# chen-bowen/instacart_next_order_recommendation

Hardware: AMD Instinct MI355X
Metric: recommend_qps_top20_49k7_catalog (higher is better)
Workload: dtype f16x3 (f32 operands split into 2 f16 planes, 3 f16 MFMAs per product, f32 accumulate; fp32-level accuracy)

## Files before the change

### instacart_next_order_recommendation_amd/csrc/encoder.hip

```cpp
#include <stdlib.h>

#include <mutex>
#include <type_traits>
#include <vector>

#include "common.h"
#include "wt_gemm.h"
#include "encoder_x3.h"

namespace icrec {

__device__ __forceinline__ int find_seq(const int32_t* __restrict__ cu, int n_seqs, int t) {
    int lo = 0, hi = n_seqs;
    while (hi - lo > 1) {
        int mid = (lo + hi) >> 1;
        if (cu[mid] <= t) lo = mid; else hi = mid;
    }
    return lo;
}

template <int H, bool SPLIT>
__device__ __forceinline__ void ln_row(float (&v)[H / 64], const float* __restrict__ g, const float* __restrict__ b,
                                       float eps, float* __restrict__ out, _Float16* __restrict__ oh,
                                       _Float16* __restrict__ ol, int lane) {
    float s = 0.0f;
#pragma unroll
    for (int j = 0; j < H / 64; ++j) s = s + v[j];
    const float mean = wave_sum_f32(s) / (float)H;
    float q = 0.0f;
#pragma unroll
    for (int j = 0; j < H / 64; ++j) {
        float d = v[j] - mean;
        q = fmaf(d, d, q);
    }
    const float var = wave_sum_f32(q) / (float)H;
    const float rstd = 1.0f / sqrtf(var + eps);
#pragma unroll
    for (int j = 0; j < H / 64; ++j) {
        const int i = lane + 64 * j;
        const float y = fmaf((v[j] - mean) * rstd, g[i], b[i]);
        if (SPLIT) {
            _Float16 hi, lo;
            split_act(y, hi, lo);
            oh[i] = hi;
            ol[i] = lo;
        } else {
            out[i] = y;
        }
    }
}

template <int H, bool SPLIT>
__global__ __launch_bounds__(256) void embed_ln_kernel(const int32_t* __restrict__ ids,
                                                       const int32_t* __restrict__ cu, int n_seqs, int T,
                                                       const float* __restrict__ word, const float* __restrict__ pos,
                                                       const float* __restrict__ type, const float* __restrict__ g,
                                                       const float* __restrict__ b, float eps, int vocab, int max_pos,
                                                       float* __restrict__ x, _Float16* __restrict__ xh,
                                                       _Float16* __restrict__ xl) {
    const int lane = threadIdx.x & 63;
    const int t = blockIdx.x * 4 + (threadIdx.x >> 6);
    if (t >= T) return;
    const int s = find_seq(cu, n_seqs, t);
    int id = ids[t];
    id = id < 0 ? 0 : (id >= vocab ? vocab - 1 : id);
    int p = t - cu[s];
    p = p >= max_pos ? max_pos - 1 : p;
    float v[H / 64];
#pragma unroll
    for (int j = 0; j < H / 64; ++j) {
        const int i = lane + 64 * j;
        v[j] = (word[(size_t)id * H + i] + type[i]) + pos[(size_t)p * H + i];
    }
    ln_row<H, SPLIT>(v, g, b, eps, x + (size_t)t * H, xh + (size_t)t * H, xl + (size_t)t * H, lane);
}

template <int H>
__global__ __launch_bounds__(256) void add_ln_kernel(const float* __restrict__ a, float* __restrict__ x, int T,
                                                     const float* __restrict__ g, const float* __restrict__ b,
                                                     float eps, _Float16* __restrict__ xh,
                                                     _Float16* __restrict__ xl) {
    const int lane = threadIdx.x & 63;
    const int t = blockIdx.x * 4 + (threadIdx.x >> 6);
    if (t >= T) return;
    float v[H / 64];
#pragma unroll
    for (int j = 0; j < H / 64; ++j) {
        const int i = lane + 64 * j;
        v[j] = a[(size_t)t * H + i] + x[(size_t)t * H + i];
    }
    ln_row<H, false>(v, g, b, eps, x + (size_t)t * H, xh + (size_t)t * H, xl + (size_t)t * H, lane);
}

__device__ __forceinline__ float gelu_erf(float x) { return x * 0.5f * (1.0f + erff(x * 0.70710678118654752440f)); }

template <class Cfg, bool GELU>
__global__ __launch_bounds__(Cfg::THREADS, 2) void linear_kernel(const float* __restrict__ A, int M, int K,
                                                                 const float* __restrict__ W, int N,
                                                                 const float* __restrict__ bias,
                                                                 float* __restrict__ out, int n_tiles_n) {
    __shared__ __attribute__((aligned(16))) float smem[Cfg::LDS_FLOATS];
    float* As = smem;
    float* Bs = smem + Cfg::BM * LDK;
    const int lane = threadIdx.x & 63, wave = threadIdx.x >> 6;
    const int wm = wave / Cfg::WAVES_N, wn = wave % Cfg::WAVES_N;
    const int bid = xcd_remap(blockIdx.x, gridDim.x);
    const int mt = bid / n_tiles_n, nt = bid % n_tiles_n;
    const int64_t m0 = (int64_t)mt * Cfg::BM, n0 = (int64_t)nt * Cfg::BN;
    f32x16 acc[Cfg::TM][Cfg::TN];
    tile_gemm<Cfg>(acc, A, m0, M, W, n0, N, K, As, Bs);
#pragma unroll
    for (int j = 0; j < Cfg::TN; ++j) {
        const int64_t col = n0 + (wn * Cfg::TN + j) * 32 + (lane & 31);
        const float bv = col < N ? bias[col] : 0.0f;
#pragma unroll
        for (int i = 0; i < Cfg::TM; ++i)
#pragma unroll
            for (int e = 0; e < 16; ++e) {
                const int64_t row = m0 + (wm * Cfg::TM + i) * 32 + acc_row(e, lane);
                if (row < M && col < N) {
                    float v = acc[i][j][e] + bv;
                    if (GELU) v = gelu_erf(v);
                    out[row * N + col] = v;
                }
            }
    }
}

constexpr int DH = 32;
constexpr int LDQ = 36;

template <int NKT>
__global__ __launch_bounds__(NKT * 64) void attention_kernel(const float* __restrict__ qkv,
                                                             const int32_t* __restrict__ cu, int heads, int H,
                                                             float scale_log2e, float* __restrict__ ctx,
                                                             _Float16* __restrict__ ch, _Float16* __restrict__ cl) {
    __shared__ __attribute__((aligned(16))) float Ks[NKT * 32 * LDQ];
    __shared__ __attribute__((aligned(16))) float Vs[NKT * 32 * DH];
    __shared__ float Ls[NKT * 32];

    const int tid = threadIdx.x, lane = tid & 63, wave = tid >> 6;
    const int s = blockIdx.x / heads, hd = blockIdx.x % heads;
    const int t0 = cu[s], L = cu[s + 1] - t0;
    const int nkt = (L + 31) >> 5;
    if (nkt > NKT || (NKT > 1 && nkt <= NKT / 2)) return;
    const int qb0 = blockIdx.y * NKT;
    if (qb0 >= nkt) return;
    const int ld = 3 * H;

    for (int id = tid; id < nkt * 32 * 8; id += NKT * 64) {
        const int row = id >> 3, c = id & 7;
        const int rr = row < L ? row : L - 1;
        const float* src = qkv + (size_t)(t0 + rr) * ld + hd * DH + c * 4;
        const float4 kv = *reinterpret_cast<const float4*>(src + H);
        const float4 vv = *reinterpret_cast<const float4*>(src + 2 * H);
        float* kp = Ks + row * LDQ + (c >> 1) * 8 + (c & 1) * 2;
        *reinterpret_cast<float2*>(kp) = make_float2(kv.x, kv.z);
        *reinterpret_cast<float2*>(kp + 4) = make_float2(kv.y, kv.w);
        *reinterpret_cast<float4*>(Vs + row * DH + c * 4) = vv;
    }
    const int r = lane & 31, h = lane >> 5;
    const int qb = qb0 + wave;
    float4 qf[4];
    {
        int qr = qb * 32 + r;
        qr = qr < L ? qr : L - 1;
        const float4* qp = reinterpret_cast<const float4*>(qkv + (size_t)(t0 + qr) * ld + hd * DH);
#pragma unroll
        for (int kq = 0; kq < 4; ++kq) {
            const float4 a = qp[2 * kq], b = qp[2 * kq + 1];
            qf[kq] = h == 0 ? make_float4(a.x, a.z, b.x, b.z) : make_float4(a.y, a.w, b.y, b.w);
        }
    }
    __syncthreads();
    if (qb >= nkt) return;

    f32x16 o;
    if constexpr (NKT > 8) {
    auto score_tile = [&](int kt) {
        f32x16 t;
#pragma unroll
        for (int e = 0; e < 16; ++e) t[e] = 0.0f;
#pragma unroll
        for (int kq = 0; kq < 4; ++kq) {
            const float4 kf = *reinterpret_cast<const float4*>(Ks + (kt * 32 + r) * LDQ + kq * 8 + h * 4);
            t = __builtin_amdgcn_mfma_f32_32x32x2f32(kf.x, qf[kq].x, t, 0, 0, 0);
            t = __builtin_amdgcn_mfma_f32_32x32x2f32(kf.y, qf[kq].y, t, 0, 0, 0);
            t = __builtin_amdgcn_mfma_f32_32x32x2f32(kf.z, qf[kq].z, t, 0, 0, 0);
            t = __builtin_amdgcn_mfma_f32_32x32x2f32(kf.w, qf[kq].w, t, 0, 0, 0);
        }
        const bool last = kt == nkt - 1;
#pragma unroll
        for (int e = 0; e < 16; ++e) {
            float v = t[e] * scale_log2e;
            if (last && kt * 32 + acc_row(e, lane) >= L) v = -INFINITY;
            t[e] = v;
        }
        return t;
    };
    float mx = -INFINITY;
    for (int kt = 0; kt < nkt; ++kt) {
        const f32x16 t = score_tile(kt);
#pragma unroll
        for (int e = 0; e < 16; ++e) mx = fmaxf(mx, t[e]);
    }
    mx = fmaxf(mx, __shfl_xor(mx, 32, 64));
    float lsum = 0.0f;
#pragma unroll
    for (int e = 0; e < 16; ++e) o[e] = 0.0f;
    for (int kt = 0; kt < nkt; ++kt) {
        f32x16 t = score_tile(kt);
#pragma unroll
        for (int e = 0; e < 16; ++e) {
            const float p = __builtin_amdgcn_exp2f(t[e] - mx);
            t[e] = p;
            lsum = lsum + p;
        }
#pragma unroll
        for (int e = 0; e < 16; ++e) {
            const int key = kt * 32 + (e & 3) + 8 * (e >> 2) + 4 * h;
            o = __builtin_amdgcn_mfma_f32_32x32x2f32(t[e], Vs[key * DH + r], o, 0, 0, 0);
        }
    }
    {
        const float other = __shfl_xor(lsum, 32, 64);
        lsum = h == 0 ? lsum + other : other + lsum;
    }
    if (h == 0) Ls[wave * 32 + r] = lsum;
    } else {
    f32x16 sc[NKT];
#pragma unroll
    for (int kt = 0; kt < NKT; ++kt) {
#pragma unroll
        for (int e = 0; e < 16; ++e) sc[kt][e] = 0.0f;
        if (kt < nkt) {
#pragma unroll
            for (int kq = 0; kq < 4; ++kq) {
                const float4 kf = *reinterpret_cast<const float4*>(Ks + (kt * 32 + r) * LDQ + kq * 8 + h * 4);
                sc[kt] = __builtin_amdgcn_mfma_f32_32x32x2f32(kf.x, qf[kq].x, sc[kt], 0, 0, 0);
                sc[kt] = __builtin_amdgcn_mfma_f32_32x32x2f32(kf.y, qf[kq].y, sc[kt], 0, 0, 0);
                sc[kt] = __builtin_amdgcn_mfma_f32_32x32x2f32(kf.z, qf[kq].z, sc[kt], 0, 0, 0);
                sc[kt] = __builtin_amdgcn_mfma_f32_32x32x2f32(kf.w, qf[kq].w, sc[kt], 0, 0, 0);
            }
        }
    }
    float mx = -INFINITY;
#pragma unroll
    for (int kt = 0; kt < NKT; ++kt) {
        if (kt < nkt) {
            const bool last = kt == nkt - 1;
#pragma unroll
            for (int e = 0; e < 16; ++e) {
                float v = sc[kt][e] * scale_log2e;
                if (last && kt * 32 + acc_row(e, lane) >= L) v = -INFINITY;
                sc[kt][e] = v;
                mx = fmaxf(mx, v);
            }
        }
    }
    mx = fmaxf(mx, __shfl_xor(mx, 32, 64));
    float lsum = 0.0f;
#pragma unroll
    for (int kt = 0; kt < NKT; ++kt) {
        if (kt < nkt) {
#pragma unroll
            for (int e = 0; e < 16; ++e) {
                const float p = __builtin_amdgcn_exp2f(sc[kt][e] - mx);
                sc[kt][e] = p;
                lsum = lsum + p;
            }
        }
    }
    {
        const float other = __shfl_xor(lsum, 32, 64);
        lsum = h == 0 ? lsum + other : other + lsum;
    }
    if (h == 0) Ls[wave * 32 + r] = lsum;
#pragma unroll
    for (int e = 0; e < 16; ++e) o[e] = 0.0f;
#pragma unroll
    for (int kt = 0; kt < NKT; ++kt) {
        if (kt < nkt) {
#pragma unroll
            for (int e = 0; e < 16; ++e) {
                const int key = kt * 32 + (e & 3) + 8 * (e >> 2) + 4 * h;
                o = __builtin_amdgcn_mfma_f32_32x32x2f32(sc[kt][e], Vs[key * DH + r], o, 0, 0, 0);
            }
        }
    }
    }
#pragma unroll
    for (int e = 0; e < 16; ++e) {
        const int qrow = acc_row(e, lane);
        const int tq = qb * 32 + qrow;
        if (tq < L) {
            const float v = o[e] / Ls[wave * 32 + qrow];
            ctx[(size_t)(t0 + tq) * H + hd * DH + r] = v;
        }
    }
}

__global__ __launch_bounds__(1024) void seq_order_kernel(const int32_t* __restrict__ cu, int n_seqs,
                                                         int32_t* __restrict__ order) {
    constexpr int NB = ICREC_MAX_SEQLEN / 32;
    __shared__ int hist[NB];
    const int tid = threadIdx.x;
    if (tid < NB) hist[tid] = 0;
    __syncthreads();
    auto bin = [&](int s) {
        const int L = cu[s + 1] - cu[s];
        const int nkt = (L + 31) >> 5;
        return NB - (nkt < 1 ? 1 : (nkt > NB ? NB : nkt));
    };
    for (int s0 = tid; s0 < n_seqs; s0 += 1024) atomicAdd(&hist[bin(n_seqs - 1 - s0)], 1);
    __syncthreads();
    if (tid == 0) {
        int run = 0;
        for (int b = 0; b < NB; ++b) { const int c = hist[b]; hist[b] = run; run += c; }
    }
    __syncthreads();
    for (int s0 = tid; s0 < n_seqs; s0 += 1024) {
        const int s = n_seqs - 1 - s0;
        order[atomicAdd(&hist[bin(s)], 1)] = s;
    }
}

typedef _Float16 half2v __attribute__((ext_vector_type(2)));

__device__ __forceinline__ half4 lds_read_tr(const _Float16* p) {
    typedef __fp16 fp16x4 __attribute__((__vector_size__(4 * sizeof(__fp16))));
    return __builtin_bit_cast(half4, __builtin_amdgcn_ds_read_tr16_b64_v4f16(
                                         (__attribute__((address_space(3))) fp16x4*)(reinterpret_cast<uintptr_t>(p))));
}

template <int NKT>
__global__ __launch_bounds__(NKT * 64, (NKT >= 6 ? 4 : NKT == 4 ? 3 : 1)) void attention_x3_kernel(const float* __restrict__ qkv,
                                                                  const int32_t* __restrict__ cu, int heads, int H,
                                                                  float scale_log2e, float* __restrict__ ctx,
                                                                  _Float16* __restrict__ ch, _Float16* __restrict__ cl,
                                                                  const int32_t* __restrict__ order, int nlo) {
    constexpr bool RECOMP = NKT >= 6;
    __shared__ __attribute__((aligned(16))) _Float16 Kbuf[2 * NKT * 32 * 32];
    _Float16* const Kh = Kbuf;
    _Float16* const Kl = Kbuf + NKT * 32 * 32;
    __shared__ __attribute__((aligned(16))) _Float16 Vh[NKT * 32 * 32];
    __shared__ __attribute__((aligned(16))) _Float16 Vl[NKT * 32 * 32];
    __shared__ float Ls[NKT * 32];
    _Float16* const Ob = Kbuf;

    const int tid = threadIdx.x, lane = tid & 63, wave = tid >> 6;
    const int sidx = blockIdx.x / heads, hd = blockIdx.x % heads;
    const int s = order != nullptr ? order[sidx] : sidx;
    const int t0 = cu[s], L = cu[s + 1] - t0;
    const int nkt = (L + 31) >> 5;
    if (nkt > NKT || nkt <= nlo) return;
    const int qb0 = blockIdx.y * NKT;
    if (qb0 >= nkt) return;
    const int ld = 3 * H;

    const int r = lane & 31, h = lane >> 5;
    const int qb = qb0 + wave;
    half8 qh[2], ql[2];
    {
        int qr = qb * 32 + r;
        qr = qr < L ? qr : L - 1;
        const float* qp = qkv + (size_t)(t0 + qr) * ld + hd * DH;
#pragma unroll
        for (int ks = 0; ks < 2; ++ks) {
            const f32x4 a = *reinterpret_cast<const f32x4*>(qp + 16 * ks + 8 * h);
            const f32x4 b = *reinterpret_cast<const f32x4*>(qp + 16 * ks + 8 * h + 4);
            half4 ah, al, bh, bl;
            split_act4(a, ah, al);
            split_act4(b, bh, bl);
            qh[ks] = half8{ah[0], ah[1], ah[2], ah[3], bh[0], bh[1], bh[2], bh[3]};
            ql[ks] = half8{al[0], al[1], al[2], al[3], bl[0], bl[1], bl[2], bl[3]};
        }
    }
    constexpr int STG = NKT * 32 * 8 / (NKT * 64);
    static_assert(NKT * 32 * 8 % (NKT * 64) == 0, "staging: whole rounds");
    f32x4 kreg[STG], vreg[STG];
#pragma unroll
    for (int it = 0; it < STG; ++it) {
        const int id = tid + it * NKT * 64;
        const int key = id >> 3, c = id & 7;
        const int rr = key < L ? key : L - 1;
        const float* src = qkv + (size_t)(t0 + rr) * ld + hd * DH + c * 4;
        kreg[it] = *reinterpret_cast<const f32x4*>(src + H);
        vreg[it] = *reinterpret_cast<const f32x4*>(src + 2 * H);
    }
#pragma unroll
    for (int it = 0; it < STG; ++it) {
        const int id = tid + it * NKT * 64;
        if (id < nkt * 32 * 8) {
            const int key = id >> 3, c = id & 7;
            half4 khi, klo, vhi, vlo;
            split_act4(kreg[it], khi, klo);
            split_act4(vreg[it], vhi, vlo);
            *reinterpret_cast<half4*>(Vh + key * 32 + c * 4) = vhi;
            *reinterpret_cast<half4*>(Vl + key * 32 + c * 4) = vlo;
            const int off = key * 32 + ((((c >> 1) ^ ((key >> 2) & 3)) << 3) | ((c & 1) << 2));
            *reinterpret_cast<half4*>(Kh + off) = khi;
            *reinterpret_cast<half4*>(Kl + off) = klo;
        }
    }
    __syncthreads();
    const bool active = qb < nkt;

    auto score_tile = [&](int kt, bool hi_only = false) {
        f32x16 t;
#pragma unroll
        for (int e = 0; e < 16; ++e) t[e] = 0.0f;
        const int key = kt * 32 + r;
#pragma unroll
        for (int ks = 0; ks < 2; ++ks) {
            const int off = key * 32 + (((2 * ks + h) ^ ((key >> 2) & 3)) << 3);
            const half8 kh = *reinterpret_cast<const half8*>(Kh + off);
            const half8 kl = *reinterpret_cast<const half8*>(Kl + off);
            t = __builtin_amdgcn_mfma_f32_32x32x16_f16(kh, qh[ks], t, 0, 0, 0);
            if (hi_only) continue;
            t = __builtin_amdgcn_mfma_f32_32x32x16_f16(kh, ql[ks], t, 0, 0, 0);
            t = __builtin_amdgcn_mfma_f32_32x32x16_f16(kl, qh[ks], t, 0, 0, 0);
        }
        if (kt == nkt - 1 && kt * 32 + 32 > L) {
#pragma unroll
            for (int e = 0; e < 16; ++e)
                if (kt * 32 + acc_row(e, lane) >= L) t[e] = -INFINITY;
        }
        return t;
    };
    auto pv_tile = [&](int kt, const f32x16& pt, f32x16& o) {
#pragma unroll
        for (int ks = 0; ks < 2; ++ks) {
            half8 ph, pl;
#pragma unroll
            for (int j = 0; j < 8; j += 2) {
                half2w a, b;
                split_pair_prescaled(pt[8 * ks + j], pt[8 * ks + j + 1], a, b);
                ph[j] = a[0]; ph[j + 1] = a[1];
                pl[j] = b[0]; pl[j + 1] = b[1];
            }
            const int base = kt * 32 + 4 * h + 16 * ks;
            const int tr_at = (base + ((lane & 15) >> 2)) * 32 + 16 * ((lane >> 4) & 1) + 4 * (lane & 3);
            const half4 v0h = lds_read_tr(Vh + tr_at);
            const half4 v1h = lds_read_tr(Vh + tr_at + 8 * 32);
            const half4 v0l = lds_read_tr(Vl + tr_at);
            const half4 v1l = lds_read_tr(Vl + tr_at + 8 * 32);
            const half8 vh = {v0h[0], v0h[1], v0h[2], v0h[3], v1h[0], v1h[1], v1h[2], v1h[3]};
            const half8 vl = {v0l[0], v0l[1], v0l[2], v0l[3], v1l[0], v1l[1], v1l[2], v1l[3]};
            o = __builtin_amdgcn_mfma_f32_32x32x16_f16(ph, vh, o, 0, 0, 0);
            o = __builtin_amdgcn_mfma_f32_32x32x16_f16(ph, vl, o, 0, 0, 0);
            o = __builtin_amdgcn_mfma_f32_32x32x16_f16(pl, vh, o, 0, 0, 0);
        }
    };
    typedef float float2w __attribute__((ext_vector_type(2)));
    const float cs = scale_log2e * (1.0f / 256.0f);
    f32x16 o;
#pragma unroll
    for (int e = 0; e < 16; ++e) o[e] = 0.0f;
    if (RECOMP) {
        if (active) {
            float mx = -INFINITY;
#pragma unroll
            for (int kt = 0; kt < NKT; ++kt) {
                if (kt < nkt) {
                    const f32x16 t = score_tile(kt, true);
#pragma unroll
                    for (int e = 0; e < 16; ++e) mx = fmaxf(mx, t[e]);
                }
            }
            mx = fmaxf(mx, __shfl_xor(mx, 32, 64));
            const float shift = fmaf(-mx, cs, 10.0f);
            float2w ls2 = float2w{0.0f, 0.0f};
#pragma unroll
            for (int kt = 0; kt < NKT; ++kt) {
                if (kt < nkt) {
                    f32x16 t = score_tile(kt);
#pragma unroll
                    for (int e = 0; e < 16; ++e) t[e] = __builtin_amdgcn_exp2f(fminf(fmaf(t[e], cs, shift), 15.9f));
#pragma unroll
                    for (int e = 0; e < 16; e += 2) ls2 = ls2 + float2w{t[e], t[e + 1]};
                    pv_tile(kt, t, o);
                }
            }
            float lrow = ls2[0] + ls2[1];
            const float other = __shfl_xor(lrow, 32, 64);
            lrow = h == 0 ? lrow + other : other + lrow;
            if (h == 0) Ls[wave * 32 + r] = lrow;
        }
    } else {
    if (active) {
    f32x16 sc[NKT];
#pragma unroll
    for (int kt = 0; kt < NKT; ++kt)
        if (kt < nkt) sc[kt] = score_tile(kt);
    float mx = -INFINITY;
#pragma unroll
    for (int kt = 0; kt < NKT; ++kt) {
        if (kt < nkt) {
#pragma unroll
            for (int e = 0; e < 16; ++e) mx = fmaxf(mx, sc[kt][e]);
        }
    }
    mx = fmaxf(mx, __shfl_xor(mx, 32, 64));
    const float shift = fmaf(-mx, cs, 10.0f);
#pragma unroll
    for (int kt = 0; kt < NKT; ++kt) {
        if (kt < nkt) {
#pragma unroll
            for (int e = 0; e < 16; ++e) sc[kt][e] = __builtin_amdgcn_exp2f(fmaf(sc[kt][e], cs, shift));
        }
    }
    float2w ls2 = float2w{0.0f, 0.0f};
#pragma unroll
    for (int kt = 0; kt < NKT; ++kt) {
        if (kt < nkt) {
#pragma unroll
            for (int e = 0; e < 16; e += 2) ls2 = ls2 + float2w{sc[kt][e], sc[kt][e + 1]};
        }
    }
    float lrow = ls2[0] + ls2[1];
    {
        const float other = __shfl_xor(lrow, 32, 64);
        lrow = h == 0 ? lrow + other : other + lrow;
    }
    if (h == 0) Ls[wave * 32 + r] = lrow;

#pragma unroll
    for (int kt = 0; kt < NKT; ++kt)
        if (kt < nkt) pv_tile(kt, sc[kt], o);
    }
    }
    __syncthreads();
    if (!active) return;
    _Float16* ob = Ob + wave * (2 * 32 * 32);
#pragma unroll
    for (int e = 0; e < 16; e += 2) {
        const int q0 = acc_row(e, lane), q1 = acc_row(e + 1, lane);
        const float v0 = o[e] * (0.0625f * __builtin_amdgcn_rcpf(Ls[wave * 32 + q0]));
        const float v1 = o[e + 1] * (0.0625f * __builtin_amdgcn_rcpf(Ls[wave * 32 + q1]));
        half2w hi, lo;
        split_pair_prescaled(v0 * WT_SA, v1 * WT_SA, hi, lo);
        ob[q0 * 32 + r] = hi[0];
        ob[q1 * 32 + r] = hi[1];
        ob[32 * 32 + q0 * 32 + r] = lo[0];
        ob[32 * 32 + q1 * 32 + r] = lo[1];
    }
#pragma unroll
    for (int t = 0; t < 2; ++t) {
        const int id = lane + 64 * t, qrow = id >> 2, c8 = (id & 3) * 8;
        const int tq = qb * 32 + qrow;
        if (tq < L) {
            const size_t at = (size_t)(t0 + tq) * H + hd * DH + c8;
            *reinterpret_cast<u32x4*>(ch + at) = *reinterpret_cast<const u32x4*>(ob + qrow * 32 + c8);
            *reinterpret_cast<u32x4*>(cl + at) = *reinterpret_cast<const u32x4*>(ob + 32 * 32 + qrow * 32 + c8);
        }
    }
}

template <int H, bool PLANES>
__global__ __launch_bounds__(H) void pool_norm_kernel(const float* __restrict__ x, const _Float16* __restrict__ xh,
                                                      const _Float16* __restrict__ xl, const int32_t* __restrict__ cu,
                                                      int n_norm, float* __restrict__ out) {
    auto at = [&](size_t idx) { return PLANES ? ((float)xh[idx] + (float)xl[idx]) * (1.0f / WT_SA) : x[idx]; };
    __shared__ float v[H];
    __shared__ float den_s;
    const int s = blockIdx.x, i = threadIdx.x;
    const int t0 = cu[s], t1 = cu[s + 1];
    float acc = 0.0f;
    int t = t0;
    for (; t + 8 <= t1; t += 8) {
        float v[8];
#pragma unroll
        for (int u = 0; u < 8; ++u) v[u] = at((size_t)(t + u) * H + i);
#pragma unroll
        for (int u = 0; u < 8; ++u) acc = acc + v[u];
    }
    for (; t < t1; ++t) acc = acc + at((size_t)t * H + i);
    float cnt = (float)(t1 - t0);
    cnt = cnt < 1e-9f ? 1e-9f : cnt;
    float val = acc / cnt;
    for (int rep = 0; rep < n_norm; ++rep) {
        v[i] = val;
        __syncthreads();
        if (i < 64) {
            float a = 0.0f;
#pragma unroll
            for (int j = 0; j < H / 64; ++j) a = fmaf(v[i + 64 * j], v[i + 64 * j], a);
            const float nrm = sqrtf(wave_sum_f32(a));
            if (i == 0) den_s = nrm > 1e-12f ? nrm : 1e-12f;
        }
        __syncthreads();
        val = val / den_s;
        __syncthreads();
    }
    out[(size_t)s * H + i] = val;
}

constexpr int HID = 384;

struct LayerW {
    float *Wqkv, *bqkv, *Wo, *bo, *g1, *b1n, *W1, *b1, *W2, *b2, *g2, *b2n;
    _Float16 *Wqkv_p, *Wo_p, *W1_p, *W2_p;
};
struct Encoder {
    icrec_bert_cfg cfg;
    int device = 0;
    int n_cu = 256;
    int max_seqlen = 256;
    float* blob = nullptr;
    float* extra = nullptr;
    _Float16* planes = nullptr;
    float *word, *pos, *type, *eg, *eb;
    LayerW layers[64];
    bool fuse = true, side_stream = true;
    int small_m = 3584;
    int tail_m = 2560;
    struct Side {
        hipStream_t caller = nullptr, side = nullptr;
        hipEvent_t ev = nullptr;
    };
    std::mutex side_mu;
    std::vector<Side*> sides;
};

static int side_for(Encoder* e, hipStream_t caller, Encoder::Side** out) {
    std::lock_guard<std::mutex> lock(e->side_mu);
    *out = nullptr;
    for (Encoder::Side* sd : e->sides)
        if (sd->caller == caller) { *out = sd; return ICREC_OK; }
    hipStreamCaptureStatus cap = hipStreamCaptureStatusNone;
    if (caller && hipStreamIsCapturing(caller, &cap) == hipSuccess && cap != hipStreamCaptureStatusNone)
        return ICREC_OK;
    Encoder::Side* sd = new Encoder::Side();
    sd->caller = caller;
    ICREC_HIP(hipStreamCreateWithFlags(&sd->side, hipStreamNonBlocking));
    ICREC_HIP(hipEventCreateWithFlags(&sd->ev, hipEventDisableTiming));
    e->sides.push_back(sd);
    *out = sd;
    return ICREC_OK;
}

static size_t weight_count(const icrec_bert_cfg* c) {
    const size_t H = c->hidden, I = c->intermediate;
    const size_t emb = (size_t)c->vocab_size * H + (size_t)c->max_position * H + (size_t)c->type_vocab * H + 2 * H;
    const size_t per = 4 * (H * H + H) + 2 * H + (I * H + I) + (H * I + H) + 2 * H;
    return emb + per * c->layers;
}

struct EncWs {
    size_t x, xs, qkv, ctx, t1, h, total;
};
static EncWs enc_ws(const icrec_bert_cfg& c, int64_t T) {
    auto al = [](size_t b) { return (b + 255) & ~(size_t)255; };
    EncWs w;
    size_t o = 0;
    w.x = o;   o += al((size_t)T * c.hidden * 4);
    w.xs = o;  o += al((size_t)T * c.hidden * 4);
    w.qkv = o; o += al((size_t)T * 3 * c.hidden * 4);
    w.ctx = o; o += al((size_t)T * c.hidden * 4);
    w.t1 = o;  o += al((size_t)T * c.hidden * 4);
    w.h = o;   o += al((size_t)T * c.intermediate * 4);
    w.total = o;
    return w;
}

struct EncBufs {
    float *x, *qkv, *ctx, *t1, *h;
    _Float16 *xh, *xl, *ch, *cl, *hh, *hl;
};

typedef TileCfg<2, 2, 2, 2> GemmBig;
constexpr long long SMALL_M_MAX = 1 << 20;

static int env_knob(const char* name, int fallback, long long hi) {
    const char* s = getenv(name);
    if (!s) return fallback;
    char* end = nullptr;
    const long long v = strtoll(s, &end, 10);
    if (end == s) return fallback;
    return (int)(v < 0 ? 0 : v > hi ? hi : v);
}

template <bool GELU>
static void launch_linear(const float* A, int M, int K, const float* W, int N, const float* bias, float* out,
                          hipStream_t st) {
    const int mt = (M + GemmBig::BM - 1) / GemmBig::BM, nt = (N + GemmBig::BN - 1) / GemmBig::BN;
    hipLaunchKernelGGL((linear_kernel<GemmBig, GELU>), dim3(mt * nt), dim3(GemmBig::THREADS), 0, st, A, M, K, W, N,
                       bias, out, nt);
}

template <int EPI>
static void launch_wt_linear(const _Float16* Xh, const _Float16* Xl, int T, int K, const _Float16* Wp, int N,
                             const float* bias, float* out, _Float16* oh, _Float16* ol, hipStream_t st, bool small) {
    if (small) {
        if constexpr (EPI == 0 || EPI == 2) {
            const int nbn = N / 64;
            auto kern = K % 256 == 0 && K >= 1024 ? wt_linear_half_kernel<EPI, 8> : wt_linear_half_kernel<EPI, 6>;
            hipLaunchKernelGGL(kern, dim3(((T + 31) / 32) * nbn), dim3(256), 0, st, Xh, Xl, T, K, Wp, N, bias, out,
                               (const _Float16*)oh, (const _Float16*)ol, nbn);
        } else {
            const int nbn = N / 128;
            hipLaunchKernelGGL((wt_linear_kernel<1, 1, 4, EPI>), dim3(((T + 31) / 32) * nbn), dim3(256), 0, st, Xh, Xl, T, K,
                               Wp, N, bias, out, oh, ol, nbn);
        }
    } else {
        const int nbn = N / 384;
        hipLaunchKernelGGL((wt_linear_kernel<3, 2, 1, EPI>), dim3(((T + 63) / 64) * nbn), dim3(256), 0, st, Xh, Xl, T, K,
                           Wp, N, bias, out, oh, ol, nbn);
    }
}

enum AttBucket { ATT_9_16, ATT_1, ATT_2, ATT_3_4, ATT_5_6, ATT_7_8, ATT_5_8, ATT_N };
constexpr int ATT_LO[ATT_N] = {9, 1, 2, 3, 5, 7, 5}, ATT_HI[ATT_N] = {16, 1, 2, 4, 6, 8, 8};

template <bool X3>
static void launch_attention(unsigned mask, const icrec_bert_cfg& c, const EncBufs& b, const int32_t* cu, int n_seqs,
                             int max_seqlen, const int32_t* order, hipStream_t st) {
    const int nkt_max = (max_seqlen + 31) / 32;
    const bool single = n_seqs == 1, split_5_8 = X3 && !single;
    const float sl2e = (1.0f / sqrtf((float)DH)) * 1.44269504088896340736f;
    for (int k = 0; k < ATT_N; ++k) {
        if (!(mask >> k & 1) || (split_5_8 ? k == ATT_5_8 : k == ATT_5_6 || k == ATT_7_8) || nkt_max < ATT_LO[k] ||
            (single && nkt_max > ATT_HI[k]))
            continue;
        const dim3 grid(n_seqs * c.heads, 1), block(ATT_HI[k] * 64);
        if constexpr (X3) {
            static const decltype(&attention_x3_kernel<1>) kern[ATT_N] = {
                attention_x3_kernel<16>, attention_x3_kernel<1>, attention_x3_kernel<2>, attention_x3_kernel<4>,
                attention_x3_kernel<6>, attention_x3_kernel<8>, attention_x3_kernel<8>};
            hipLaunchKernelGGL(kern[k], grid, block, 0, st, b.qkv, cu, c.heads, c.hidden, sl2e, b.ctx, b.ch, b.cl, order,
                               ATT_LO[k] - 1);
        } else {
            static const decltype(&attention_kernel<1>) kern[ATT_N] = {
                attention_kernel<16>, attention_kernel<1>, attention_kernel<2>, attention_kernel<4>, nullptr, nullptr,
                attention_kernel<8>};
            hipLaunchKernelGGL(kern[k], grid, block, 0, st, b.qkv, cu, c.heads, c.hidden, sl2e, b.ctx, b.ch, b.cl);
        }
    }
}

}

using namespace icrec;

extern "C" {

size_t icrec_encoder_weight_count(const icrec_bert_cfg* cfg) { return cfg ? weight_count(cfg) : 0; }

int icrec_encoder_create(const float* weights_host, size_t n_floats, const icrec_bert_cfg* cfg, int device,
                         icrec_encoder** out) {
    ICREC_REQUIRE(weights_host && cfg && out, "icrec_encoder_create: NULL argument");
    ICREC_REQUIRE(cfg->hidden == HID, "icrec_encoder_create: this build supports hidden=384 only (got %d)", cfg->hidden);
    ICREC_REQUIRE(cfg->heads * DH == cfg->hidden, "icrec_encoder_create: head_dim must be 32 (heads=%d)", cfg->heads);
    ICREC_REQUIRE(cfg->intermediate >= 384 && cfg->intermediate % 384 == 0, "icrec_encoder_create: intermediate size must be a multiple of 384 (got %d)", cfg->intermediate);
    ICREC_REQUIRE(cfg->layers >= 1 && cfg->layers <= 64, "icrec_encoder_create: layers must be in [1,64]");
    ICREC_REQUIRE(cfg->vocab_size >= 1 && cfg->max_position >= 1 && cfg->type_vocab >= 1, "icrec_encoder_create: bad vocab/position sizes");
    ICREC_REQUIRE(cfg->n_normalize >= 0 && cfg->n_normalize <= 4, "icrec_encoder_create: n_normalize must be in [0,4]");
    ICREC_REQUIRE(cfg->gemm_mode == ICREC_GEMM_F32 || cfg->gemm_mode == ICREC_GEMM_F16X3, "icrec_encoder_create: unknown gemm_mode %d", cfg->gemm_mode);
    ICREC_REQUIRE(n_floats == weight_count(cfg), "icrec_encoder_create: weight blob has %zu floats, expected %zu", n_floats, weight_count(cfg));
    ICREC_HIP(hipSetDevice(device));
    hipDeviceProp_t prop;
    ICREC_HIP(hipGetDeviceProperties(&prop, device));
    if (strncmp(prop.gcnArchName, "gfx950", 6) != 0) {
        set_error("icrec_encoder_create: device %d is %s, this library is built for gfx950 only", device, prop.gcnArchName);
        return ICREC_ENODEV;
    }
    Encoder* e = new Encoder();
    e->cfg = *cfg;
    e->device = device;
    e->n_cu = prop.multiProcessorCount > 0 ? prop.multiProcessorCount : 256;
    e->max_seqlen = cfg->max_position < 256 ? cfg->max_position : 256;
    {
        const char* fuse_env = getenv("ICREC_FUSE");
        const char* side_env = getenv("ICREC_SIDE_STREAM");
        e->fuse = !(fuse_env && fuse_env[0] == '0');
        e->small_m = env_knob("ICREC_SMALL_M", e->small_m, SMALL_M_MAX);
        e->tail_m = env_knob("ICREC_TAIL_M", e->tail_m, 64LL * e->n_cu - 1);
        e->side_stream = !(side_env && side_env[0] == '0');
    }
    const size_t H = cfg->hidden, I = cfg->intermediate;
    const size_t mat_per_layer = 3 * H * H + H * H + I * H + H * I;
    const bool x3 = cfg->gemm_mode == ICREC_GEMM_F16X3;
    if (hipMalloc(&e->blob, n_floats * 4) != hipSuccess ||
        hipMalloc(&e->extra, (size_t)cfg->layers * (3 * H * H + 3 * H) * 4) != hipSuccess ||
        (x3 && hipMalloc(&e->planes, (size_t)cfg->layers * mat_per_layer * 2 * sizeof(_Float16)) != hipSuccess)) {
        set_error("icrec_encoder_create: hipMalloc failed");
        if (e->blob) (void)hipFree(e->blob);
        if (e->extra) (void)hipFree(e->extra);
        delete e;
        return ICREC_ENOMEM;
    }
    ICREC_HIP(hipMemcpy(e->blob, weights_host, n_floats * 4, hipMemcpyHostToDevice));
    float* p = e->blob;
    e->word = p; p += (size_t)cfg->vocab_size * H;
    e->pos = p;  p += (size_t)cfg->max_position * H;
    e->type = p; p += (size_t)cfg->type_vocab * H;
    e->eg = p;   p += H;
    e->eb = p;   p += H;
    float* x = e->extra;
    _Float16* pl = e->planes;
    auto pack = [&](const float* w, int N, int K, _Float16*& out) {
        out = pl;
        pl += (size_t)2 * N * K;
        hipLaunchKernelGGL(pack_weights_kernel, dim3(1024), dim3(256), 0, 0, w, N, K, out);
    };
    for (int l = 0; l < cfg->layers; ++l) {
        LayerW& L = e->layers[l];
        L.Wqkv = x; x += 3 * H * H;
        L.bqkv = x; x += 3 * H;
        for (int part = 0; part < 3; ++part) {
            ICREC_HIP(hipMemcpy(L.Wqkv + part * H * H, p, H * H * 4, hipMemcpyDeviceToDevice)); p += H * H;
            ICREC_HIP(hipMemcpy(L.bqkv + part * H, p, H * 4, hipMemcpyDeviceToDevice)); p += H;
        }
        L.Wo = p; p += H * H; L.bo = p; p += H;
        L.g1 = p; p += H; L.b1n = p; p += H;
        L.W1 = p; p += I * H; L.b1 = p; p += I;
        L.W2 = p; p += H * I; L.b2 = p; p += H;
        L.g2 = p; p += H; L.b2n = p; p += H;
        if (x3) {
            pack(L.Wqkv, (int)(3 * H), (int)H, L.Wqkv_p);
            pack(L.Wo, (int)H, (int)H, L.Wo_p);
            pack(L.W1, (int)I, (int)H, L.W1_p);
            pack(L.W2, (int)H, (int)I, L.W2_p);
        }
    }
    ICREC_HIP(hipGetLastError());
    ICREC_HIP(hipDeviceSynchronize());
    *out = reinterpret_cast<icrec_encoder*>(e);
    return ICREC_OK;
}

int icrec_encoder_destroy(icrec_encoder* h) {
    Encoder* e = reinterpret_cast<Encoder*>(h);
    if (!e) return ICREC_OK;
    (void)hipSetDevice(e->device);
    (void)hipFree(e->blob);
    (void)hipFree(e->extra);
    if (e->planes) (void)hipFree(e->planes);
    for (Encoder::Side* sd : e->sides) {
        (void)hipStreamSynchronize(sd->side);
        (void)hipStreamDestroy(sd->side);
        (void)hipEventDestroy(sd->ev);
        delete sd;
    }
    delete e;
    return ICREC_OK;
}

int icrec_encoder_set_max_seqlen(icrec_encoder* h, int32_t max_seqlen) {
    Encoder* e = reinterpret_cast<Encoder*>(h);
    ICREC_REQUIRE(e, "icrec_encoder_set_max_seqlen: NULL encoder");
    const int hi = e->cfg.max_position < ICREC_MAX_SEQLEN ? e->cfg.max_position : ICREC_MAX_SEQLEN;
    ICREC_REQUIRE(max_seqlen >= 1 && max_seqlen <= hi, "icrec_encoder_set_max_seqlen: max_seqlen must be in [1, %d] (got %d)", hi, max_seqlen);
    e->max_seqlen = max_seqlen;
    return ICREC_OK;
}

size_t icrec_encode_workspace_bytes(const icrec_encoder* h, int64_t total_tokens, int32_t n_seqs) {
    const Encoder* e = reinterpret_cast<const Encoder*>(h);
    if (!e || total_tokens < 1 || n_seqs < 1) return 0;
    return enc_ws(e->cfg, total_tokens).total;
}

static int batch_tail(const Encoder* e, int T) {
    const int round_tokens = 64 * e->n_cu;
    return T > round_tokens && T % round_tokens <= e->tail_m ? T % round_tokens : 0;
}

int icrec_encode_batch_split(const icrec_encoder* h, int64_t total_tokens, int64_t* main_tokens, int64_t* tail_tokens) {
    const Encoder* e = reinterpret_cast<const Encoder*>(h);
    ICREC_REQUIRE(e && main_tokens && tail_tokens && total_tokens >= 1 && total_tokens < (1ll << 31), "icrec_encode_batch_split: bad argument");
    *tail_tokens = batch_tail(e, (int)total_tokens);
    *main_tokens = total_tokens - *tail_tokens;
    return ICREC_OK;
}

static const int32_t* embed(const Encoder* e, const EncBufs& b, const int32_t* ids_dev, const int32_t* cu_dev,
                            int n_seqs, int T, hipStream_t st) {
    const icrec_bert_cfg& c = e->cfg;
    const bool x3 = c.gemm_mode == ICREC_GEMM_F16X3;
    int32_t* order = nullptr;
    if (x3 && n_seqs >= 64 && e->fuse) {
        order = reinterpret_cast<int32_t*>(b.x);
        hipLaunchKernelGGL(seq_order_kernel, dim3(1), dim3(1024), 0, st, cu_dev, n_seqs, order);
    }
    hipLaunchKernelGGL((x3 ? embed_ln_kernel<HID, true> : embed_ln_kernel<HID, false>), dim3((T + 3) / 4), dim3(256), 0,
                       st, ids_dev, cu_dev, n_seqs, T, e->word, e->pos, e->type, e->eg, e->eb, c.ln_eps, c.vocab_size,
                       c.max_position, b.x, b.xh, b.xl);
    return order;
}

static hipError_t link(const Encoder::Side* sd, hipStream_t from, hipStream_t to) {
    const hipError_t err = hipEventRecord(sd->ev, from);
    return err != hipSuccess ? err : hipStreamWaitEvent(to, sd->ev, 0);
}

struct Range {
    int r0, n;
    hipStream_t st;
    bool small;
    bool layer;
    bool fold;
    Range(const Encoder* e, int r0, int n, hipStream_t st)
        : r0(r0), n(n), st(st), small(n <= e->small_m), layer(e->fuse && !small), fold(e->fuse && small) {}
    bool launches_qkv(int l) const { return l == 0 || !layer; }
    bool ffn_ln_to_next(int l, int layers) const { return fold && l + 1 < layers; }
};

static int encode_x3(Encoder* e, const EncBufs& b, const int32_t* cu_dev, int n_seqs, int T, int max_seqlen,
                     const int32_t* order, hipStream_t st) {
    const icrec_bert_cfg& c = e->cfg;
    const int H = c.hidden, I = c.intermediate;
    const bool split_att = e->side_stream && n_seqs >= 64 && max_seqlen > 128;
    const int T_tail = batch_tail(e, T), T_main = T - T_tail;
    Encoder::Side* sd = nullptr;
    if (e->side_stream && (T_tail || split_att))
        if (int rc_ = side_for(e, st, &sd)) return rc_;
    const Range main(e, 0, T_main, st), tail(e, T_main, T_tail, sd ? sd->side : st);
    const bool tail_on_side = T_tail && sd;
    if (main.layer || tail.layer) {
        if (int rc_ = ensure_dynamic_lds(reinterpret_cast<const void*>(qkv_resident_kernel), QKVR_LDS)) return rc_;
        if (int rc_ = ensure_dynamic_lds(reinterpret_cast<const void*>(ffn_fused2_kernel), FFN2_LDS)) return rc_;
    }

    auto qkv_stage = [&](const Range& r, int l) {
        const LayerW& L = e->layers[l];
        _Float16 *const xhr = b.xh + (size_t)r.r0 * H, *const xlr = b.xl + (size_t)r.r0 * H;
        float* const qkvr = b.qkv + (size_t)r.r0 * 3 * H;
        if (r.layer) {
            hipLaunchKernelGGL(qkv_resident_kernel, dim3((r.n + 63) / 64), dim3(512), QKVR_LDS, r.st, xhr, xlr, r.n,
                               L.Wqkv_p, L.bqkv, qkvr, 3 * H);
        } else if (l > 0 && r.ffn_ln_to_next(l - 1, c.layers)) {
            const LayerW& Lp = e->layers[l - 1];
            const int nbn = 3 * H / 64;
            hipLaunchKernelGGL((wt_linear_lnin_kernel<0>), dim3(((r.n + 31) / 32) * nbn), dim3(256), 0, r.st,
                               (const float*)(b.t1 + (size_t)r.r0 * H), r.n, Lp.g2, Lp.b2n, c.ln_eps, xhr, xlr, L.Wqkv_p,
                               3 * H, L.bqkv, qkvr, (_Float16*)nullptr, (_Float16*)nullptr, nbn);
        } else {
            launch_wt_linear<0>(xhr, xlr, r.n, H, L.Wqkv_p, 3 * H, L.bqkv, qkvr, nullptr, nullptr, r.st, r.small);
        }
    };
    auto post_stage = [&](const Range& r, int l) {
        const LayerW& L = e->layers[l];
        float* const t1r = b.t1 + (size_t)r.r0 * H;
        _Float16 *const xhr = b.xh + (size_t)r.r0 * H, *const xlr = b.xl + (size_t)r.r0 * H;
        const _Float16 *const chr = b.ch + (size_t)r.r0 * H, *const clr = b.cl + (size_t)r.r0 * H;
        if (r.layer) {
            ScopedTimer tm(T_FFN_UP, r.st);
            const bool next_qkv = l + 1 < c.layers;
            const LayerW& Ln = e->layers[next_qkv ? l + 1 : l];
            hipLaunchKernelGGL(ffn_fused2_kernel, dim3((r.n + 63) / 64), dim3(512), FFN2_LDS, r.st, xhr, xlr, r.n, I,
                               L.W1_p, L.b1, L.W2_p, L.b2, L.g2, L.b2n, c.ln_eps, chr, clr, L.Wo_p, L.bo, L.g1, L.b1n,
                               next_qkv ? (const _Float16*)Ln.Wqkv_p : (const _Float16*)nullptr, (const float*)Ln.bqkv,
                               b.qkv + (size_t)r.r0 * 3 * H, 3 * H);
            return;
        }
        _Float16 *const hhr = b.hh + (size_t)r.r0 * I, *const hlr = b.hl + (size_t)r.r0 * I;
        launch_wt_linear<2>(chr, clr, r.n, H, L.Wo_p, H, L.bo, t1r, xhr, xlr, r.st, r.small);
        if (r.fold) {
            const int nbn = I / 64;
            hipLaunchKernelGGL((wt_linear_lnin_kernel<1>), dim3(((r.n + 31) / 32) * nbn), dim3(256), 0, r.st,
                               (const float*)t1r, r.n, L.g1, L.b1n, c.ln_eps, xhr, xlr, L.W1_p, I, L.b1, (float*)nullptr,
                               hhr, hlr, nbn);
        } else {
            hipLaunchKernelGGL(ln_wt_kernel, dim3((r.n + 15) / 16), dim3(256), 0, r.st, t1r, r.n, L.g1, L.b1n, c.ln_eps,
                               xhr, xlr);
            ScopedTimer tm(r.small ? T_NSLOTS - 1 : T_FFN_UP, r.st);
            launch_wt_linear<1>(xhr, xlr, r.n, H, L.W1_p, I, L.b1, nullptr, hhr, hlr, r.st, r.small);
        }
        launch_wt_linear<2>(hhr, hlr, r.n, I, L.W2_p, H, L.b2, t1r, xhr, xlr, r.st, r.small);
        if (!r.ffn_ln_to_next(l, c.layers))
            hipLaunchKernelGGL(ln_wt_kernel, dim3((r.n + 15) / 16), dim3(256), 0, r.st, t1r, r.n, L.g2, L.b2n, c.ln_eps,
                               xhr, xlr);
    };

    if (tail_on_side) ICREC_HIP(link(sd, st, sd->side));
    for (int l = 0; l < c.layers; ++l) {
        if (T_tail && tail.launches_qkv(l)) qkv_stage(tail, l);
        if (main.launches_qkv(l)) qkv_stage(main, l);
        if (tail_on_side) ICREC_HIP(link(sd, sd->side, st));
        if (split_att && sd) {
            ICREC_HIP(link(sd, st, sd->side));
            const unsigned side_buckets = 1u << ATT_1 | 1u << ATT_2 | 1u << ATT_3_4 | 1u << ATT_7_8;
            launch_attention<true>(1u << ATT_9_16, c, b, cu_dev, n_seqs, max_seqlen, order, st);
            launch_attention<true>(side_buckets, c, b, cu_dev, n_seqs, max_seqlen, order, sd->side);
            launch_attention<true>(1u << ATT_5_6, c, b, cu_dev, n_seqs, max_seqlen, order, st);
            ICREC_HIP(link(sd, sd->side, st));
        } else {
            launch_attention<true>(~0u, c, b, cu_dev, n_seqs, max_seqlen, order, st);
        }
        if (tail_on_side) ICREC_HIP(link(sd, st, sd->side));
        if (T_tail) post_stage(tail, l);
        post_stage(main, l);
    }
    if (tail_on_side) ICREC_HIP(link(sd, sd->side, st));
    return ICREC_OK;
}

static int encode_f32(const Encoder* e, const EncBufs& b, const int32_t* cu_dev, int n_seqs, int T, int max_seqlen,
                      hipStream_t st) {
    const icrec_bert_cfg& c = e->cfg;
    const int H = c.hidden, I = c.intermediate, rows_grid = (T + 3) / 4;
    for (int l = 0; l < c.layers; ++l) {
        const LayerW& L = e->layers[l];
        launch_linear<false>(b.x, T, H, L.Wqkv, 3 * H, L.bqkv, b.qkv, st);
        launch_attention<false>(~0u, c, b, cu_dev, n_seqs, max_seqlen, nullptr, st);
        launch_linear<false>(b.ctx, T, H, L.Wo, H, L.bo, b.t1, st);
        hipLaunchKernelGGL(add_ln_kernel<HID>, dim3(rows_grid), dim3(256), 0, st, b.t1, b.x, T, L.g1, L.b1n,
                           c.ln_eps, b.xh, b.xl);
        {
            ScopedTimer tm(T_FFN_UP, st);
            launch_linear<true>(b.x, T, H, L.W1, I, L.b1, b.h, st);
        }
        launch_linear<false>(b.h, T, I, L.W2, H, L.b2, b.t1, st);
        hipLaunchKernelGGL(add_ln_kernel<HID>, dim3(rows_grid), dim3(256), 0, st, b.t1, b.x, T, L.g2, L.b2n,
                           c.ln_eps, b.xh, b.xl);
    }
    return ICREC_OK;
}

int icrec_encode(icrec_encoder* h, const int32_t* ids_dev, const int32_t* cu_dev, int32_t n_seqs, int64_t T64,
                 int32_t max_seqlen, float* out_dev, void* ws, size_t ws_bytes, void* stream) {
    Encoder* e = reinterpret_cast<Encoder*>(h);
    ICREC_REQUIRE(e && ids_dev && cu_dev && out_dev, "icrec_encode: NULL argument");
    ICREC_REQUIRE(n_seqs >= 1 && T64 >= n_seqs && T64 < (1ll << 31), "icrec_encode: bad n_seqs/total_tokens (%d, %lld)", n_seqs, (long long)T64);
    ICREC_REQUIRE(max_seqlen >= 1 && max_seqlen <= e->max_seqlen, "icrec_encode: max_seqlen must be in [1, %d] (got %d)", e->max_seqlen, max_seqlen);
    const int T = (int)T64;
    const EncWs w = enc_ws(e->cfg, T);
    if (!ws || ws_bytes < w.total) {
        set_error("icrec_encode: workspace too small (%zu < %zu)", ws_bytes, w.total);
        return ICREC_ENOMEM;
    }
    ICREC_HIP(hipSetDevice(e->device));
    hipStream_t st = (hipStream_t)stream;
    ScopedTimer whole(T_ENCODE, st);
    char* base = reinterpret_cast<char*>(ws);
    const icrec_bert_cfg& c = e->cfg;
    const int H = c.hidden, I = c.intermediate;
    const bool x3 = c.gemm_mode == ICREC_GEMM_F16X3;
    EncBufs b;
    b.x = reinterpret_cast<float*>(base + w.x);
    b.qkv = reinterpret_cast<float*>(base + w.qkv);
    b.ctx = reinterpret_cast<float*>(base + w.ctx);
    b.t1 = reinterpret_cast<float*>(base + w.t1);
    b.h = reinterpret_cast<float*>(base + w.h);
    b.xh = reinterpret_cast<_Float16*>(base + w.xs);
    b.xl = b.xh + (size_t)T * H;
    b.ch = reinterpret_cast<_Float16*>(b.ctx);
    b.cl = b.ch + (size_t)T * H;
    b.hh = reinterpret_cast<_Float16*>(b.h);
    b.hl = b.hh + (size_t)T * I;
    const int32_t* order = embed(e, b, ids_dev, cu_dev, n_seqs, T, st);
    if (int rc_ = x3 ? encode_x3(e, b, cu_dev, n_seqs, T, max_seqlen, order, st)
                     : encode_f32(e, b, cu_dev, n_seqs, T, max_seqlen, st))
        return rc_;
    hipLaunchKernelGGL((x3 ? pool_norm_kernel<HID, true> : pool_norm_kernel<HID, false>), dim3(n_seqs), dim3(HID), 0, st,
                       b.x, b.xh, b.xl, cu_dev, c.n_normalize, out_dev);
    ICREC_HIP(hipGetLastError());
    return ICREC_OK;
}

}
```

Measured before the change: 109,200.

## Fuse embedding+LayerNorm into first-layer QKV kernel and overlap seq ordering on side stream

Result: no change. 109,600, median of 6 (+0.4%).

```diff
diff --git a/instacart_next_order_recommendation_amd/csrc/encoder.hip b/instacart_next_order_recommendation_amd/csrc/encoder.hip
--- a/instacart_next_order_recommendation_amd/csrc/encoder.hip
+++ b/instacart_next_order_recommendation_amd/csrc/encoder.hip
@@ -57,9 +57,9 @@
                                                        const float* __restrict__ type, const float* __restrict__ g,
                                                        const float* __restrict__ b, float eps, int vocab, int max_pos,
                                                        float* __restrict__ x, _Float16* __restrict__ xh,
-                                                       _Float16* __restrict__ xl) {
+                                                       _Float16* __restrict__ xl, int t0 = 0) {
     const int lane = threadIdx.x & 63;
-    const int t = blockIdx.x * 4 + (threadIdx.x >> 6);
+    const int t = t0 + blockIdx.x * 4 + (threadIdx.x >> 6);
     if (t >= T) return;
     const int s = find_seq(cu, n_seqs, t);
     int id = ids[t];
@@ -73,6 +73,67 @@
         v[j] = (word[(size_t)id * H + i] + type[i]) + pos[(size_t)p * H + i];
     }
     ln_row<H, SPLIT>(v, g, b, eps, x + (size_t)t * H, xh + (size_t)t * H, xl + (size_t)t * H, lane);
+}
+
+__global__ __launch_bounds__(512, 2) void embed_qkv_kernel(const int32_t* __restrict__ ids,
+                                                           const int32_t* __restrict__ cu, int n_seqs, int T,
+                                                           const float* __restrict__ word, const float* __restrict__ pos,
+                                                           const float* __restrict__ type, const float* __restrict__ eg,
+                                                           const float* __restrict__ eb, float eps, int vocab,
+                                                           int max_pos, _Float16* __restrict__ xh,
+                                                           _Float16* __restrict__ xl, const _Float16* __restrict__ Wp,
+                                                           const float* __restrict__ bias, float* __restrict__ out,
+                                                           int N) {
+    constexpr int H = 384, NTOK = 64 / 8;
+    extern __shared__ __attribute__((aligned(16))) char smem2[];
+    char* const Xs = smem2;
+    const int tid = threadIdx.x, lane = tid & 63, wave = wave_uniform(tid >> 6), c = lane & 15, g = lane >> 4;
+    float* const stg = reinterpret_cast<float*>(smem2 + FFN2_X_BYTES + wave * QKVR_STG_BYTES);
+    const int64_t m0 = (int64_t)blockIdx.x * 64;
+    const int tw = (int)m0 + wave * NTOK;
+    float* const par = reinterpret_cast<float*>(smem2 + FFN2_X_BYTES);
+    if (tid < 192) *reinterpret_cast<f32x4*>(par + 4 * tid) = wt_ln_par_load(eg, eb, tid);
+    int id = 0, p = 0;
+    if (lane < NTOK) {
+        const int t = tw + lane < T ? tw + lane : T - 1;
+        id = ids[t];
+        id = id < 0 ? 0 : (id >= vocab ? vocab - 1 : id);
+        p = t - cu[find_seq(cu, n_seqs, t)];
+        p = p >= max_pos ? max_pos - 1 : p;
+    }
+    float v[NTOK][H / 64];
+#pragma unroll
+    for (int k = 0; k < NTOK; ++k) {
+        const int ik = __builtin_amdgcn_readlane(id, k), pk = __builtin_amdgcn_readlane(p, k);
+#pragma unroll
+        for (int j = 0; j < H / 64; ++j) {
+            const int i = lane + 64 * j;
+            v[k][j] = (word[(size_t)ik * H + i] + type[i]) + pos[(size_t)pk * H + i];
+        }
+    }
+    bar_lds();
+#pragma unroll
+    for (int k = 0; k < NTOK; ++k) {
+        _Float16* const row = reinterpret_cast<_Float16*>(Xs + (wave * NTOK + k) * 768);
+        ln_row<H, true>(v[k], par, par + H, eps, nullptr, row, row + FFN2_XPLANE / 2, lane);
+    }
+    lds_order();
+    constexpr int NR = 2 * NTOK * 48 / 64;
+    u32x4 o[NR];
+#pragma unroll
+    for (int r = 0; r < NR; ++r) {
+        const int idx = lane + 64 * r, pl = idx / (NTOK * 48), k = idx / 48 % NTOK, ch = idx % 48;
+        o[r] = *reinterpret_cast<const u32x4*>(Xs + pl * FFN2_XPLANE + (wave * NTOK + k) * 768 + ch * 16);
+    }
+    lds_order();
+#pragma unroll
+    for (int r = 0; r < NR; ++r) {
+        const int idx = lane + 64 * r, pl = idx / (NTOK * 48), k = idx / 48 % NTOK, ch = idx % 48;
+        *reinterpret_cast<u32x4*>(Xs + pl * FFN2_XPLANE + ffn_x_pos(wave * NTOK + k, ch)) = o[r];
+        if (tw + k < T) *reinterpret_cast<u32x4*>((pl ? xl : xh) + (int64_t)(tw + k) * H + ch * 8) = o[r];
+    }
+    __syncthreads();
+    qkv_block_walk(Xs, stg, Wp, bias, out, N, m0, T, wave, lane, c, g, lane * 8);
 }
 
 template <int H>
@@ -875,19 +936,13 @@
     return ICREC_OK;
 }
 
-static const int32_t* embed(const Encoder* e, const EncBufs& b, const int32_t* ids_dev, const int32_t* cu_dev,
-                            int n_seqs, int T, hipStream_t st) {
+static void embed(const Encoder* e, const EncBufs& b, const int32_t* ids_dev, const int32_t* cu_dev, int n_seqs, int t0,
+                  int T, hipStream_t st) {
     const icrec_bert_cfg& c = e->cfg;
     const bool x3 = c.gemm_mode == ICREC_GEMM_F16X3;
-    int32_t* order = nullptr;
-    if (x3 && n_seqs >= 64 && e->fuse) {
-        order = reinterpret_cast<int32_t*>(b.x);
-        hipLaunchKernelGGL(seq_order_kernel, dim3(1), dim3(1024), 0, st, cu_dev, n_seqs, order);
-    }
-    hipLaunchKernelGGL((x3 ? embed_ln_kernel<HID, true> : embed_ln_kernel<HID, false>), dim3((T + 3) / 4), dim3(256), 0,
-                       st, ids_dev, cu_dev, n_seqs, T, e->word, e->pos, e->type, e->eg, e->eb, c.ln_eps, c.vocab_size,
-                       c.max_position, b.x, b.xh, b.xl);
-    return order;
+    hipLaunchKernelGGL((x3 ? embed_ln_kernel<HID, true> : embed_ln_kernel<HID, false>), dim3((T - t0 + 3) / 4),
+                       dim3(256), 0, st, ids_dev, cu_dev, n_seqs, T, e->word, e->pos, e->type, e->eg, e->eb, c.ln_eps,
+                       c.vocab_size, c.max_position, b.x, b.xh, b.xl, t0);
 }
 
 static hipError_t link(const Encoder::Side* sd, hipStream_t from, hipStream_t to) {
@@ -907,19 +962,23 @@
     bool ffn_ln_to_next(int l, int layers) const { return fold && l + 1 < layers; }
 };
 
-static int encode_x3(Encoder* e, const EncBufs& b, const int32_t* cu_dev, int n_seqs, int T, int max_seqlen,
-                     const int32_t* order, hipStream_t st) {
+static int encode_x3(Encoder* e, const EncBufs& b, const int32_t* ids_dev, const int32_t* cu_dev, int n_seqs, int T,
+                     int max_seqlen, hipStream_t st) {
     const icrec_bert_cfg& c = e->cfg;
     const int H = c.hidden, I = c.intermediate;
     const bool split_att = e->side_stream && n_seqs >= 64 && max_seqlen > 128;
     const int T_tail = batch_tail(e, T), T_main = T - T_tail;
+    const Range main(e, 0, T_main, st);
+    int32_t* const order = e->fuse && n_seqs >= 64 ? reinterpret_cast<int32_t*>(b.x) : nullptr;
     Encoder::Side* sd = nullptr;
-    if (e->side_stream && (T_tail || split_att))
+    if (e->side_stream && (T_tail || split_att || (main.layer && order)))
         if (int rc_ = side_for(e, st, &sd)) return rc_;
-    const Range main(e, 0, T_main, st), tail(e, T_main, T_tail, sd ? sd->side : st);
+    const Range tail(e, T_main, T_tail, sd ? sd->side : st);
     const bool tail_on_side = T_tail && sd;
+    const bool pre_on_side = main.layer && sd;
     if (main.layer || tail.layer) {
         if (int rc_ = ensure_dynamic_lds(reinterpret_cast<const void*>(qkv_resident_kernel), QKVR_LDS)) return rc_;
+        if (int rc_ = ensure_dynamic_lds(reinterpret_cast<const void*>(embed_qkv_kernel), QKVR_LDS)) return rc_;
         if (int rc_ = ensure_dynamic_lds(reinterpret_cast<const void*>(ffn_fused2_kernel), FFN2_LDS)) return rc_;
     }
 
@@ -927,7 +986,11 @@
         const LayerW& L = e->layers[l];
         _Float16 *const xhr = b.xh + (size_t)r.r0 * H, *const xlr = b.xl + (size_t)r.r0 * H;
         float* const qkvr = b.qkv + (size_t)r.r0 * 3 * H;
-        if (r.layer) {
+        if (r.layer && l == 0 && r.r0 == 0) {
+            hipLaunchKernelGGL(embed_qkv_kernel, dim3((r.n + 63) / 64), dim3(512), QKVR_LDS, r.st, ids_dev, cu_dev, n_seqs,
+                               r.n, e->word, e->pos, e->type, e->eg, e->eb, c.ln_eps, c.vocab_size, c.max_position, b.xh,
+                               b.xl, L.Wqkv_p, L.bqkv, qkvr, 3 * H);
+        } else if (r.layer) {
             hipLaunchKernelGGL(qkv_resident_kernel, dim3((r.n + 63) / 64), dim3(512), QKVR_LDS, r.st, xhr, xlr, r.n,
                                L.Wqkv_p, L.bqkv, qkvr, 3 * H);
         } else if (l > 0 && r.ffn_ln_to_next(l - 1, c.layers)) {
@@ -974,11 +1037,20 @@
                                xhr, xlr);
     };
 
-    if (tail_on_side) ICREC_HIP(link(sd, st, sd->side));
+    if (main.layer) {
+        const hipStream_t pre = pre_on_side ? sd->side : st;
+        if (pre_on_side) ICREC_HIP(link(sd, st, sd->side));
+        if (order) hipLaunchKernelGGL(seq_order_kernel, dim3(1), dim3(1024), 0, pre, cu_dev, n_seqs, order);
+        if (T_tail) embed(e, b, ids_dev, cu_dev, n_seqs, T_main, T, tail.st);
+    } else {
+        if (order) hipLaunchKernelGGL(seq_order_kernel, dim3(1), dim3(1024), 0, st, cu_dev, n_seqs, order);
+        embed(e, b, ids_dev, cu_dev, n_seqs, 0, T, st);
+        if (tail_on_side) ICREC_HIP(link(sd, st, sd->side));
+    }
     for (int l = 0; l < c.layers; ++l) {
         if (T_tail && tail.launches_qkv(l)) qkv_stage(tail, l);
         if (main.launches_qkv(l)) qkv_stage(main, l);
-        if (tail_on_side) ICREC_HIP(link(sd, sd->side, st));
+        if (tail_on_side || (l == 0 && pre_on_side)) ICREC_HIP(link(sd, sd->side, st));
         if (split_att && sd) {
             ICREC_HIP(link(sd, st, sd->side));
             const unsigned side_buckets = 1u << ATT_1 | 1u << ATT_2 | 1u << ATT_3_4 | 1u << ATT_7_8;
@@ -1050,8 +1122,8 @@
     b.cl = b.ch + (size_t)T * H;
     b.hh = reinterpret_cast<_Float16*>(b.h);
     b.hl = b.hh + (size_t)T * I;
-    const int32_t* order = embed(e, b, ids_dev, cu_dev, n_seqs, T, st);
-    if (int rc_ = x3 ? encode_x3(e, b, cu_dev, n_seqs, T, max_seqlen, order, st)
+    if (!x3) embed(e, b, ids_dev, cu_dev, n_seqs, 0, T, st);
+    if (int rc_ = x3 ? encode_x3(e, b, ids_dev, cu_dev, n_seqs, T, max_seqlen, st)
                      : encode_f32(e, b, cu_dev, n_seqs, T, max_seqlen, st))
         return rc_;
     hipLaunchKernelGGL((x3 ? pool_norm_kernel<HID, true> : pool_norm_kernel<HID, false>), dim3(n_seqs), dim3(HID), 0, st,
```
